# MohamedAtwan/AirCraftOptimalControl

Measured on AMD Instinct MI355X. Metric: Newton iters/sec (whole node), batched 6-state T=500 trajectories; fp64 rel-err, higher is better.
Workload: dtype f64

## Files before the change

### aircraftoptimalcontrol_amd/_lib.py

```python
import ctypes as C
import os
import subprocess

_PKG = os.path.dirname(os.path.abspath(__file__))
_SO = os.environ.get("AOC_LIB") or os.path.join(_PKG, "lib", "libaoc_hip.so")
_SRC = [os.path.join(_PKG, "csrc", f) for f in ("aoc_kernels.hip", "aoc_device.h", "aoc_passes.inc")]
_SRC += sorted(os.path.join(_PKG, "csrc", "passes", f) for f in os.listdir(os.path.join(_PKG, "csrc", "passes")) if f.endswith(".inc"))
_HDR = os.path.join(os.path.dirname(_PKG), "include", "aoc.h")

AOC_TILE = 64
AOC_ENS_NSTAT = 16
AOC_ENV_NREC = 44
AOC_ABI_VERSION = 5

ST_NAN, ST_VNONPOS, ST_SINGULAR, ST_REGULARISED, ST_ARMIJO_EXH, ST_CONVERGED = 1, 2, 4, 8, 16, 32


class AocError(RuntimeError):
    pass


def library_path():
    return _SO


def build_library(force=False, verbose=False):
    deps = _SRC + [_HDR]
    if not force and os.path.exists(_SO) and all(os.path.getmtime(_SO) >= os.path.getmtime(d) for d in deps):
        return _SO
    os.makedirs(os.path.dirname(_SO), exist_ok=True)
    hipcc = os.environ.get("HIPCC", "/opt/rocm/bin/hipcc")
    cmd = [hipcc, "--offload-arch=gfx950", "-O3", "-std=c++17", "-fPIC", "-shared", _SRC[0], "-o", _SO]
    if verbose:
        print(" ".join(cmd))
    subprocess.check_call(cmd)
    return _SO


class Model(C.Structure):
    _fields_ = [(n, C.c_double) for n in ("cd0", "cda", "cla", "m", "g", "S", "rho", "J", "dt")]


class Problem(C.Structure):
    _fields_ = [("model", Model), ("QQt", C.c_double * 36), ("RRt", C.c_double * 4), ("QQT", C.c_double * 36),
                ("B", C.c_int32), ("T", C.c_int32), ("x_in_f32", C.c_int32), ("x_out_f32", C.c_int32),
                ("ref_per_traj", C.c_int32), ("ref_T", C.c_int32), ("x_is_rollout", C.c_int32), ("reserved", C.c_int32),
                ("ref", C.c_void_p), ("stream", C.c_void_p)]


class Params(C.Structure):
    _fields_ = [("max_iters", C.c_int32), ("armijo_maxiters", C.c_int32), ("stepsize_0", C.c_double),
                ("cc", C.c_double), ("beta", C.c_double), ("term_cond", C.c_double),
                ("hessian_switch", C.c_int32), ("reserved", C.c_int32)]


class MpcNoise(C.Structure):
    _fields_ = [("seed", C.c_uint64), ("step", C.c_uint32), ("first", C.c_uint32), ("sigma", C.c_double * 6)]


class Tuning(C.Structure):
    _fields_ = [(n, C.c_int32) for n in ("nspec", "split_tiles", "split_bw_tiles", "fw_lin", "ls_wcap", "ls_kgrow",
                                         "trial_split", "solve_norepack", "ls_worklist", "ls_cpl", "ls_depth_min",
                                         "fw_recompute", "store_candidates", "bw4_tiles", "bw5", "solve_repack_pct",
                                         "solve_sync_fast", "solve_split_tiles", "track_hcut", "bw_hcut", "fw_wpe1",
                                         "hcut_chain6", "bw_hcut_full", "fw_duo", "hcut_waves", "hcut_pairs")]


_P, _I, _D, _Z = C.c_void_p, C.c_int32, C.c_double, C.c_size_t
SYMBOLS = {
    "aoc_get_tuning": (None, [_P]),
    "aoc_set_tuning": (None, [_P]),
    "aoc_version": (C.c_char_p, []),
    "aoc_strerror": (C.c_char_p, [C.c_int]),
    "aoc_last_hip_error": (C.c_char_p, []),
    "aoc_tiled_elems": (_Z, [_I, _I, _I]),
    "aoc_ntiles": (_I, [_I]),
    "aoc_pack": (C.c_int, [_I, _I, _I, _P, _P, _P]),
    "aoc_unpack": (C.c_int, [_I, _I, _I, _P, _P, _P]),
    "aoc_pack_f32": (C.c_int, [_I, _I, _I, _P, _P, _P]),
    "aoc_unpack_f32": (C.c_int, [_I, _I, _I, _P, _P, _P]),
    "aoc_step_batch": (C.c_int, [_P, _I] + [_P] * 10),
    "aoc_cost_batch": (C.c_int, [_P, _I] + [_P] * 10),
    "aoc_traj_cost": (C.c_int, [_P, _P, _P, _P, _P]),
    "aoc_initial_trajectory": (C.c_int, [_P, _D, _D, _P, _P, _P]),
    "aoc_rollout_cost": (C.c_int, [_P] * 9),
    "aoc_backward": (C.c_int, [_P, _I] + [_P] * 7 + [_Z]),
    "aoc_backward_scratch_bytes": (_Z, [_I, _I]),
    "aoc_gradient": (C.c_int, [_P] * 7),
    "aoc_forward": (C.c_int, [_P, _P, _I] + [_P] * 9 + [_Z, _P]),
    "aoc_candidate_bytes": (_Z, [_I, _I, _I]),
    "aoc_default_ncand": (_I, [_I, _I, _I]),
    "aoc_linesearch_scratch_bytes": (_Z, [_I, _I]),
    "aoc_spec_max": (_I, []),
    "aoc_default_nspec": (_I, [_I, _I]),
    "aoc_linesearch": (C.c_int, [_P, _P, _I] + [_P] * 13 + [_Z, _P, _Z]),
    "aoc_linesearch_search": (C.c_int, [_P, _P, _I] + [_P] * 9 + [_Z]),
    "aoc_linesearch_update": (C.c_int, [_P] * 12 + [_Z, _I, _P, _P, _Z]),
    "aoc_lqr_tracking": (C.c_int, [_P] * 9),
    "aoc_ltv_lqr": (C.c_int, [_I, _I, _I] + [_P] * 17),
    "aoc_workspace_bytes": (_Z, [_I, _I]),
    "aoc_newton_iterate": (C.c_int, [_P, _P, _I] + [_P] * 5 + [_Z] + [_P] * 7),
    "aoc_solve_workspace_bytes": (_Z, [_I, _I]),
    "aoc_newton_solve": (C.c_int, [_P] * 6 + [_Z, _I] + [_P] * 10),
    "aoc_newton_solve2": (C.c_int, [_P] * 6 + [_Z, _I] + [_P] * 11),
    "aoc_abi_version": (_I, []),
    "aoc_summary": (C.c_int, [_I, _P, _P, _P, _P, _I, _P]),
    "aoc_streams_concurrent": (C.c_int, [_P, _P]),
    "aoc_solve_trace": (C.c_int, [_P, _I]),
    "aoc_solve_trace_rows": (_I, []),
    "aoc_mpc_step": (C.c_int, [_P] * 3 + [_I] + [_P] * 6 + [_Z] + [_P] * 16),
    "aoc_track_ensemble": (C.c_int, [_P, _I, _I] + [_P] * 8),
    "aoc_ensemble_envelope_scratch_bytes": (_Z, [_I, _I, _I]),
    "aoc_track_ensemble_envelope": (C.c_int, [_P, _I, _I] + [_P] * 10 + [_Z]),
    "aoc_traj_cost_f32": (C.c_int, [_P] * 5),
    "aoc_initial_trajectory_f32": (C.c_int, [_P, _D, _D, _P, _P, _P]),
    "aoc_rollout_cost_f32": (C.c_int, [_P] * 9),
    "aoc_workspace_bytes_f32": (_Z, [_I, _I]),
    "aoc_newton_iterate_f32": (C.c_int, [_P, _P, _I] + [_P] * 5 + [_Z] + [_P] * 7),
# ... 70 lines not shown
```

### aircraftoptimalcontrol_amd/csrc/aoc_kernels.hip

```cpp
#include <hip/hip_runtime.h>

#include <cstdarg>
#include <cstdio>
#include <cstdlib>
#include <cstring>
#include <mutex>
#include <vector>

#include "../../include/aoc.h"

namespace aoc_common {
constexpr int TILE = 64;
}
#define AOC_DEVICE_COMMON
using aoc_common::TILE;

#define AOC_DISPATCH_BOOL(flag, NAME, ...)            \
    do {                                              \
        if (flag) { constexpr bool NAME = true; __VA_ARGS__; } \
        else { constexpr bool NAME = false; __VA_ARGS__; }      \
    } while (0)
#define AOC_DISPATCH_RPT(flag, NAME, ...)                                         \
    do {                                                                          \
        if (flag) { constexpr bool NAME = sizeof(real) == 8; __VA_ARGS__; }       \
// ... 55 lines not shown
    }
    if (lane == 0) { sh[0][wv] = sc; sh[1][wv] = sd; shi[0][wv] = st; shi[1][wv] = nn; }
    __syncthreads();
    if (tid == 0) {
        double a = 0.0, b = 0.0;
        long long c = 0, d = 0;
        for (int w = 0; w < 16; w++) { a += sh[0][w]; b += sh[1][w]; c += shi[0][w]; d += shi[1][w]; }
        if (accumulate) { out[0] += a; out[1] += b; out[2] += (double)c; out[3] += (double)B; out[4] += (double)d; }
        else { out[0] = a; out[1] = b; out[2] = (double)c; out[3] = (double)B; out[4] = (double)d; }
    }
}

__global__ void k_spin(long long ticks, int* sink) {
    const long long t0 = wall_clock64();
    int n = 0;
    while (wall_clock64() - t0 < ticks && n < (1 << 24)) n++;
    if (sink && n < 0) *sink = n;
}

static thread_local char g_hip_err[256] = "";

static int check_launch(const char* what) {
    hipError_t e = hipGetLastError();
    if (e != hipSuccess) {
        snprintf(g_hip_err, sizeof g_hip_err, "%s: %s", what, hipGetErrorString(e));
        return AOC_ELAUNCH;
    }
    return AOC_OK;
}

static int einval(const char* fmt, ...) {
    va_list ap;
    va_start(ap, fmt);
    vsnprintf(g_hip_err, sizeof g_hip_err, fmt, ap);
    va_end(ap);
    return AOC_EINVAL;
}

static aoc_tuning g_tuning;
static std::once_flag g_tuning_once;

static void tuning_defaults(aoc_tuning* t) {
    auto env = [](const char* name, int dflt) { const char* e = getenv(name); return e && *e ? atoi(e) : dflt; };
    memset(t, 0, sizeof *t);
    t->nspec = env("AOC_NSPEC", 0);
    t->split_tiles = env("AOC_SPLIT_TILES", 512);
    t->split_bw_tiles = env("AOC_SPLIT_BW_TILES", 512);
    t->fw_lin = env("AOC_FW_LIN", -1);
    t->ls_wcap = env("AOC_LS_WCAP", 0);
    t->ls_kgrow = env("AOC_LS_KGROW", 0);
    t->trial_split = env("AOC_TRIAL_SPLIT", 1);
    t->solve_norepack = env("AOC_SOLVE_NOREPACK", 0);
    t->ls_worklist = env("AOC_LS_WORKLIST", -1);
    t->ls_cpl = env("AOC_LS_CPL", 1);
    t->ls_depth_min = env("AOC_LS_DEPTH_MIN", 2);
    t->fw_recompute = env("AOC_FW_RECOMPUTE", 1);
    t->store_candidates = env("AOC_STORE_CANDIDATES", 1);
    t->bw4_tiles = env("AOC_BW4_TILES", 256);
    t->bw5 = env("AOC_BW5", 1);
    t->solve_repack_pct = env("AOC_SOLVE_REPACK_PCT", 70);
    t->solve_sync_fast = env("AOC_SOLVE_SYNC_FAST", 2);
    t->solve_split_tiles = env("AOC_SOLVE_SPLIT_TILES", 2048);
    t->track_hcut = env("AOC_TRACK_HCUT", -1);
    t->bw_hcut = env("AOC_BW_HCUT", -1);
    t->fw_wpe1 = env("AOC_FW_WPE1", 1);
    t->hcut_chain6 = env("AOC_HCUT_CHAIN6", 0);
    t->bw_hcut_full = env("AOC_BW_HCUT_FULL", 2);
    t->fw_duo = env("AOC_FW_DUO", 1);
    t->hcut_waves = env("AOC_HCUT_WAVES", 1);
    t->hcut_pairs = env("AOC_HCUT_PAIRS", 1);
}

static const aoc_tuning& tuning() {
    std::call_once(g_tuning_once, [] { tuning_defaults(&g_tuning); });
    return g_tuning;
}

static bool is_diag(const double* M, int n) {
    for (int i = 0; i < n; i++)
        for (int j = 0; j < n; j++)
            if (i != j && M[i * n + j] != 0.0) return false;
    return true;
}

static int check_problem(const aoc_problem* p) {
    if (!p) return einval("aoc_problem is NULL");
    if (!p->ref) return einval("aoc_problem.ref (reference curves) is NULL");
    if (p->B < 1 || p->T < 3) return einval("aoc_problem: B = %d, T = %d (need B >= 1, T >= 3)", p->B, p->T);
    if (p->ref_per_traj && p->ref_T != 0 && p->ref_T < p->T)
        return einval("aoc_problem: ref_T = %d < T = %d (samples per trajectory of the per-trajectory reference array)", p->ref_T, p->T);
    if (p->RRt[1] != p->RRt[2])
        return einval("aoc_problem.RRt is not symmetric (R01 = %g, R10 = %g): the 2x2 gain solve needs R = R^T", p->RRt[1],
                      p->RRt[2]);
    return AOC_OK;
}

static int check_riccati_weights(const aoc_problem* p, const char* who) {
    const struct { const double* M; const char* name; } w[2] = {{p->QQt, "QQt"}, {p->QQT, "QQT"}};
    for (const auto& m : w)
        for (int i = 0; i < 6; i++)
            for (int j = i + 1; j < 6; j++)
                if (m.M[i * 6 + j] != m.M[j * 6 + i])
                    return einval("%s: aoc_problem.%s is not symmetric (%s[%d][%d] = %.17g, %s[%d][%d] = %.17g): the Riccati "
                                  "recursion needs Q = Q^T and Q_T = Q_T^T", who, m.name, m.name, i, j, m.M[i * 6 + j], m.name,
                                  j, i, m.M[j * 6 + i]);
    return AOC_OK;
}
// ... 308 lines not shown
```

### aircraftoptimalcontrol_amd/csrc/passes/api.inc

```
static KConst make_const(const aoc_model& md, const double* Q, const double* R, const double* QT, int B, int T) {
    KConst k;
    memset(&k, 0, sizeof k);
    k.cd0 = (real)md.cd0; k.cda = (real)md.cda; k.cla = (real)md.cla; k.m = (real)md.m; k.g = (real)md.g; k.S = (real)md.S;
    k.rho = (real)md.rho;
    k.J = (real)md.J; k.dt = (real)md.dt;
    k.dtm = (real)(md.dt / md.m);
    k.mg = (real)(md.m * md.g);
    k.hrho = (real)(0.5 * md.rho);
    k.krs = (real)(md.rho * md.S);
    k.b41 = (real)(md.dt / md.J);
    k.rJ = R(1.0) / k.J;
    for (int i = 0; i < 36; i++) { if (Q) k.Q[i] = (real)Q[i]; if (QT) k.QT[i] = (real)QT[i]; }
    for (int i = 0; i < 4; i++) if (R) k.R[i] = (real)R[i];
    k.B = B; k.T = T; k.ntiles = (B + TILE - 1) / TILE;
    k.refT = T; k.rpt = 0;
    k.diag = (Q && R && QT) ? (is_diag(Q, 6) && is_diag(R, 2) && is_diag(QT, 6)) : 1;
    return k;
}

static KConst make_const(const aoc_problem* p) {
    KConst k = make_const(p->model, p->QQt, p->RRt, p->QQT, p->B, p->T);
    k.rpt = p->ref_per_traj != 0;
    if (k.rpt && p->ref_T > 0) k.refT = p->ref_T;
    return k;
// ... 194 lines not shown
    hipLaunchKernelGGL((k_forward<D, RP, N, XR, XT>), dim3(k.ntiles), dim3(TILE), 0, st, k, *prm, (const real*)p->ref, \
                       (const XT*)x, u, x0, Kt, du, descent, J_trial, status)
#define LAUNCH_FW(N)                                                                                                \
    AOC_DISPATCH_DR(k, D, RP, do {                                                                                  \
        if (!p->x_in_f32) LAUNCH_FW_(N, false, real);                                                               \
        else if (xrc) LAUNCH_FW_(N, true, float);                                                                   \
        else LAUNCH_FW_(N, false, float);                                                                           \
    } while (0))
#define LAUNCH_FW_ROLES(KERNEL, GROUPS, NWAVES)                                                                      \
    hipLaunchKernelGGL(KERNEL, dim3(k.ntiles, GROUPS), dim3((NWAVES) * TILE), 0, st, k, *prm, n_spec, cb,           \
                       (const real*)p->ref, (const XT*)x, u, x0, Kt, du, descent, J_trial, status, ntrials_hint)
    const bool xrc = p->x_is_rollout && p->x_in_f32 && tuning().fw_recompute != 0;
    const int split_env = tuning().split_tiles;
    const int split_fw = split_env;
    if (n_spec > 3 || (k.ntiles <= split_fw && p->T >= 3)) {
        if (p->T < 3) return AOC_EINVAL;
        const CandBuf cb = cand_carve(cand, p->B, p->T, n_spec);
        const int one_per_cu = tuning().fw_wpe1 ? 256 : 0;
        const int fw_lin = tuning().fw_lin;
        const int duo_max = tuning().fw_duo == 1 ? 256 : tuning().fw_duo;
        if (duo_max > 0 && n_spec > FWS_TPG && k.ntiles * ((n_spec + 1) / 2) <= duo_max) {
            AOC_DISPATCH_DR(k, D, RP, AOC_DISPATCH_XT(p->x_in_f32, XT,
                LAUNCH_FW_ROLES((k_forward_duo<D, RP, XT>), (n_spec + FWD_CPG - 1) / FWD_CPG, 8)));
        } else if (fw_lin > 0 || (fw_lin < 0 && n_spec <= FWL_TPG)) {
            const int ngroups = (n_spec + FWL_TPG - 1) / FWL_TPG;
            AOC_DISPATCH_DR(k, D, RP, AOC_DISPATCH_XT(p->x_in_f32, XT, AOC_DISPATCH_WPE(k.ntiles * ngroups <= one_per_cu, WPE,
                LAUNCH_FW_ROLES((k_forward_lin<D, RP, XT, WPE>), ngroups, 2 + FWL_TPG))));
        } else {
            const int ngroups = (n_spec + FWS_TPG - 1) / FWS_TPG;
            const int nwaves = 1 + (n_spec < FWS_TPG ? n_spec : FWS_TPG);
            AOC_DISPATCH_DR(k, D, RP, AOC_DISPATCH_XT(p->x_in_f32, XT, AOC_DISPATCH_WPE(k.ntiles * ngroups <= one_per_cu, WPE,
                LAUNCH_FW_ROLES((k_forward_split<D, RP, XT, WPE>), ngroups, nwaves))));
        }
    } else if (n_spec == 1) LAUNCH_FW(1);
    else if (n_spec == 2) LAUNCH_FW(2);
    else LAUNCH_FW(3);
#undef LAUNCH_FW_ROLES
#undef LAUNCH_FW
#undef LAUNCH_FW_
    return check_launch("k_forward");
}

static size_t ls_layout(int ntiles, void* scratch, LsScratch* sc) {
    const size_t nt = (size_t)ntiles;
    size_t off = 0;
    auto take = [&](size_t bytes) { char* q = scratch ? (char*)scratch + off : nullptr; off += align_up(bytes, 16); return q; };
    LsScratch s;
    s.mask = (unsigned long long*)take(nt * sizeof(unsigned long long));
    s.prefix = (int*)take((nt + 1) * sizeof(int));
    s.first_ok = (int*)take(nt * TILE * sizeof(int));
    s.st = (LsState*)take(sizeof(aoc64::LsState));
    s.items = (int2*)take(nt * TILE * LS_WL_IPL * sizeof(int2));
    s.next_r = (int*)take(nt * TILE * sizeof(int));
    s.wl_count = (int*)take(2 * LS_WL_ROUNDS * sizeof(int));
    if (sc) *sc = s;
    return off;
}

static bool ls_use_worklist(int ntiles) {
    const aoc_tuning& tn = tuning();
    return tn.ls_worklist > 0 || (tn.ls_worklist < 0 && ntiles > tn.split_tiles);
}

static int api_ls_search(const aoc_problem* p, const aoc_params* prm, int32_t n_spec, const real* u, const real* x0,
                         const real* du, const real* J_cur, const real* descent, const real* J_trial0, real* stepsize,
                         int32_t* ntrials, void* scratch, size_t scratch_size, LsFrozen frozen = LsFrozen{nullptr, nullptr}) {
    int rc = check_problem(p);
    if (rc) return rc;
    if (!prm || !u || !x0 || !du || !J_cur || !descent || (!J_trial0 && n_spec > 0) || !stepsize || !ntrials || !scratch)
        return einval("aoc_linesearch: NULL argument");
    if (scratch_size < aoc_linesearch_scratch_bytes(p->B, p->T))
        return einval("aoc_linesearch: scratch of %zu bytes, %zu needed (aoc_linesearch_scratch_bytes)", scratch_size,
                      aoc_linesearch_scratch_bytes(p->B, p->T));
    if (prm->armijo_maxiters < 1 || prm->armijo_maxiters >= LS_MAX_STEPS)
        return einval("aoc_linesearch: armijo_maxiters = %d (1 .. %d)", prm->armijo_maxiters, LS_MAX_STEPS - 1);
    if (n_spec < 0 || n_spec > AOC_SPEC_MAX) return einval("aoc_linesearch: n_spec = %d (0 .. %d)", n_spec, AOC_SPEC_MAX);
    KConst k = make_const(p);
    hipStream_t st = (hipStream_t)p->stream;
    LsScratch sc;
    ls_layout(k.ntiles, scratch, &sc);
    const aoc_tuning& tn = tuning();
    if (ls_use_worklist(k.ntiles)) {
        const int cpl = tn.ls_cpl >= 4 ? 4 : tn.ls_cpl >= 2 ? 2 : 1;
        if (prm->armijo_maxiters > 255) return einval("aoc_linesearch: armijo_maxiters > 255");
        const int remaining = prm->armijo_maxiters > n_spec ? prm->armijo_maxiters - n_spec : 0;
        const int per_round = LS_WL_IPL * cpl;
        const int nrounds = remaining > 0 ? 1 + (remaining + per_round - 1) / per_round : 0;
        if (nrounds > LS_WL_ROUNDS)
            return einval("aoc_linesearch: armijo_maxiters = %d needs more than %d work-list rounds", prm->armijo_maxiters,
                          LS_WL_ROUNDS);
        if (hipMemsetAsync(sc.wl_count, 0, 2 * LS_WL_ROUNDS * sizeof(int), st) != hipSuccess)
            return check_launch("aoc_linesearch");
        hipLaunchKernelGGL(k_ls_init_wl, dim3(k.ntiles), dim3(TILE), 0, st, *prm, n_spec, cpl,
                           tn.ls_depth_min > 1 ? tn.ls_depth_min : 1, k.ntiles * TILE, J_cur, descent, J_trial0, stepsize,
                           ntrials, sc, frozen);
        const int ipl = (remaining + cpl - 1) / cpl < LS_WL_IPL ? (remaining + cpl - 1) / cpl : LS_WL_IPL;
        const int wcap = tn.ls_wcap > 0 ? tn.ls_wcap : 2048;
        for (int r = 0; r < nrounds; r++) {
            if (r == 0)
                hipLaunchKernelGGL(k_ls_plan_wl, dim3(k.ntiles), dim3(TILE), 0, st, prm->armijo_maxiters, n_spec, cpl,
                                   wcap * TILE, sc);
            else
                hipLaunchKernelGGL(k_ls_replan, dim3(k.ntiles), dim3(TILE), 0, st, prm->armijo_maxiters, cpl, r, stepsize,
                                   ntrials, sc);
#define LAUNCH_WL(C, PINNED)                                                                                      \
    AOC_DISPATCH_DR(k, D, RP,                                                                                  \
        hipLaunchKernelGGL((k_ls_trial_wl<D, RP, C, PINNED>), dim3(k.ntiles * ipl), dim3(TILE), 0, st, k, *prm, r,    \
                           (const real*)p->ref, u, x0, du, J_cur, descent, sc))
            if (cpl == 4) LAUNCH_WL(4, false);
            else if (cpl == 2) LAUNCH_WL(2, false);
            else {
                LAUNCH_WL(1, true);
                LAUNCH_WL(1, false);
            }
#undef LAUNCH_WL
        }
        return check_launch("aoc_linesearch");
    }
    const int wcap_env = tn.ls_wcap > 0 ? tn.ls_wcap : 1024;
    const int kgrow_set = tn.ls_kgrow;
    const int kgrow_env = kgrow_set > 0 ? kgrow_set : (k.ntiles <= 512 ? 9 : 1);
    const int wcap = k.ntiles > wcap_env ? k.ntiles : wcap_env;
    const bool trial_split = tn.trial_split != 0 && p->T >= 3;
    hipLaunchKernelGGL(k_ls_init, dim3(k.ntiles), dim3(TILE), 0, st, *prm, n_spec, k.ntiles * TILE, J_cur, descent,
                       J_trial0, stepsize, ntrials, sc, frozen);
    const int remaining = prm->armijo_maxiters - n_spec;
    int nrounds = remaining < LS_ROUNDS ? remaining : LS_ROUNDS;
    if (nrounds > 1 && (long)k.ntiles * remaining <= wcap_env && kgrow_env + 1 >= remaining) nrounds = 1;
    for (int r = 0; r < nrounds; r++) {
        const int last = (r == nrounds - 1);
        if (r > 0) hipLaunchKernelGGL(k_ls_resolve, dim3(k.ntiles), dim3(TILE), 0, st, sc, stepsize, ntrials);
        hipLaunchKernelGGL(k_ls_plan, dim3(1), dim3(1024), 0, st, k.ntiles, prm->armijo_maxiters, wcap_env, kgrow_env,
                           last, sc);
        const int grid = last ? k.ntiles * (remaining > 1 ? remaining : 1) : wcap;
        if (trial_split && k.ntiles <= 512) {
            AOC_DISPATCH_DR(k, D, RP,
                hipLaunchKernelGGL((k_ls_trial_split<D, RP>), dim3(grid), dim3(2 * TILE), 0, st, k, *prm, (const real*)p->ref, u,
                                   x0, du, J_cur, descent, sc));
        } else {
            AOC_DISPATCH_DR(k, D, RP,
                hipLaunchKernelGGL((k_ls_trial<D, RP>), dim3(grid), dim3(TILE), 0, st, k, *prm, (const real*)p->ref, u, x0, du,
                                   J_cur, descent, sc));
        }
    }
    return check_launch("aoc_linesearch");
}

static int api_ls_update(const aoc_problem* p, const aoc_params* prm, const real* u, const real* x0, const real* du,
                         void* x_new, real* u_new, real* J_new, real* stepsize, int32_t* ntrials, int32_t* status,
                         void* scratch, size_t scratch_size, int32_t n_spec = 0, const real* J_trial = nullptr,
                         const void* cand = nullptr, size_t cand_size = 0) {
    int rc = check_problem(p);
    if (rc) return rc;
    if (!prm || !u || !x0 || !du || !x_new || !u_new || !J_new || !stepsize || !ntrials || !scratch)
        return einval("aoc_linesearch: NULL argument");
    if (scratch_size < aoc_linesearch_scratch_bytes(p->B, p->T))
        return einval("aoc_linesearch: scratch of %zu bytes, %zu needed (aoc_linesearch_scratch_bytes)", scratch_size,
                      aoc_linesearch_scratch_bytes(p->B, p->T));
    if (cand && J_trial && (n_spec < 1 || n_spec > AOC_SPEC_MAX || cand_size < cand_bytes(p->B, p->T, n_spec)))
        return einval("aoc_linesearch: candidate store of %zu bytes for n_spec = %d, %zu needed (aoc_candidate_bytes)", cand_size,
                      n_spec, n_spec >= 1 && n_spec <= AOC_SPEC_MAX ? cand_bytes(p->B, p->T, n_spec) : (size_t)0);
    if (prm->armijo_maxiters < 1 || prm->armijo_maxiters >= LS_MAX_STEPS)
        return einval("aoc_linesearch: armijo_maxiters = %d (1 .. %d)", prm->armijo_maxiters, LS_MAX_STEPS - 1);
    KConst k = make_const(p);
    hipStream_t st = (hipStream_t)p->stream;
    LsScratch sc;
    ls_layout(k.ntiles, scratch, &sc);
// ... 159 lines not shown
```

### aircraftoptimalcontrol_amd/csrc/passes/linesearch.inc

```
constexpr int LS_MAX_STEPS = 64;
constexpr int LS_NOT_FOUND = 0x7fffffff;
#ifndef AOC_LS_ROUNDS
#define AOC_LS_ROUNDS 4
#endif
constexpr int LS_ROUNDS = AOC_LS_ROUNDS;

constexpr int LS_WL_IPL = 8;
constexpr int LS_WL_ROUNDS = 16;

struct LsState {
    int r_next;
    int r_start;
    int K;
    int count;
    int nw;
    int round;
    int scheme;
    int pad;
    real alpha[LS_MAX_STEPS];
};

struct LsScratch {
    unsigned long long* mask;
    int* prefix;
    int* first_ok;
    LsState* st;
    int2* items;
    int* next_r;
    int* wl_count;
};

struct LsFrozen { const int* orig; const int* ret; };

__global__ __launch_bounds__(TILE) void k_ls_init(aoc_params prm, int nspec, int Bp, const real* __restrict__ J_cur,
                                                  const real* __restrict__ descent,
                                                  const real* __restrict__ J_trial, real* __restrict__ stepsize,
                                                  int* __restrict__ ntrials, LsScratch sc, LsFrozen frozen) {
    const int tile = blockIdx.x, lane = threadIdx.x, b = tile * TILE + lane;
    const real JP = J_cur[b], d = descent[b];
    real a = prm.stepsize_0;
    bool searching = true;
    int ntr = 0;
    real acc = a;
    for (int j = 0; j < nspec && j < prm.armijo_maxiters; j++) {
        if (searching) {
            ntr = j + 1;
            if (!armijo_reject(J_trial[(size_t)j * Bp + b], JP, prm.cc, a, d)) { searching = false; acc = a; }
        }
        a = prm.beta * a;
    }
    if (frozen.orig) {
        const int ob = frozen.orig[b];
        if (ob < 0 || frozen.ret[ob] != -2) { searching = false; acc = R(0.0); ntr = 0; }
    }
    const unsigned long long m = __ballot(searching);
    stepsize[b] = acc;
    ntrials[b] = ntr;
    sc.first_ok[b] = LS_NOT_FOUND;
    if (lane == 0) sc.mask[tile] = m;
    if (tile == 0 && lane == 0) {
        real al = prm.stepsize_0;
        sc.st->alpha[0] = al;
        for (int i = 1; i <= prm.armijo_maxiters; i++) { al = prm.beta * al; sc.st->alpha[i] = al; }
        const int done = nspec < prm.armijo_maxiters ? nspec : prm.armijo_maxiters;
        sc.st->r_next = done;
        sc.st->r_start = done;
        sc.st->K = 0;
        sc.st->count = 0;
        sc.st->nw = 0;
        sc.st->round = 0;
        sc.st->scheme = 0;
// ... 86 lines not shown
    }
}

__device__ __forceinline__ int nth_set_bit(unsigned long long m, int rank) {
    int pos = 0;
#pragma unroll
    for (int w = 32; w >= 1; w >>= 1) {
        const unsigned long long low = m & ((1ull << w) - 1ull);
        const int c = __popcll(low);
        if (rank >= c) { rank -= c; m >>= w; pos += w; }
        else m = low;
    }
    return pos;
}

__device__ __forceinline__ void ls_locate(const LsScratch& sc, int ntiles, int j, int& tile, int& hl) {
    const int* __restrict__ prefix = sc.prefix;
    int lo = 0, hi = ntiles;
    while (hi - lo > 1) {
        const int mid = (lo + hi) >> 1;
        if (prefix[mid] <= j) lo = mid; else hi = mid;
    }
    tile = lo;
    hl = nth_set_bit(sc.mask[lo], j - prefix[lo]);
}

template <bool DIAG, bool RPT>
__global__ __launch_bounds__(TILE) void k_ls_trial(KConst k, aoc_params prm, const real* __restrict__ ref,
                                                   const real* __restrict__ u, const real* __restrict__ x0,
                                                   const real* __restrict__ du, const real* __restrict__ J_cur,
                                                   const real* __restrict__ descent, LsScratch sc) {
    const LsState* st = sc.st;
    const int K = st->K, nw = st->nw;
    const int w = blockIdx.x;
    if (w >= K * nw) return;
    const int kidx = w / nw, slot = w - kidx * nw;
    const int r = st->r_start + kidx;
    const real a_r = st->alpha[r];
    const int count = st->count;
    const int lane = threadIdx.x;
    const int first = slot * TILE;
    const bool valid = first + lane < count;
    int tile, hl;
    ls_locate(sc, k.ntiles, valid ? first + lane : count - 1, tile, hl);
    const int b = tile * TILE + hl;
    real xs[6];
#pragma unroll
    for (int c = 0; c < 6; c++) xs[c] = x0[((size_t)tile * 6 + c) * TILE + hl];
    int f2 = 0;
    const real Jt = rollout<DIAG, RPT, false, real>(k, ref, tile, hl, xs, u, du, a_r, false, nullptr, nullptr, f2);
    if (valid && !armijo_reject(Jt, J_cur[b], prm.cc, a_r, descent[b])) atomicMin(&sc.first_ok[b], r);
}

__device__ __forceinline__ void ls_put_items(const LsScratch& sc, int round, int lane, int b, int r, int depth, int cpl) {
    const int nit = (depth + cpl - 1) / cpl;
    int incl = nit;
#pragma unroll
    for (int off = 1; off < 64; off <<= 1) {
        const int v = __shfl_up(incl, off);
        if (lane >= off) incl += v;
    }
    const int total = __shfl(incl, 63);
    if (total == 0) return;
    int base = 0;
    if (lane == 63) base = atomicAdd(&sc.wl_count[round], total);
    base = __shfl(base, 63);
    int pos = base + incl - nit;
    for (int c = 0; c < nit; c++) {
        const int n = depth - c * cpl < cpl ? depth - c * cpl : cpl;
        sc.items[pos + c] = make_int2(b, (r + c * cpl) | (n << 8));
    }
}

__global__ __launch_bounds__(TILE) void k_ls_init_wl(aoc_params prm, int nspec, int cpl, int depth_min, int Bp,
                                                     const real* __restrict__ J_cur, const real* __restrict__ descent,
                                                     const real* __restrict__ J_trial, real* __restrict__ stepsize,
                                                     int* __restrict__ ntrials, LsScratch sc, LsFrozen frozen) {
    const int tile = blockIdx.x, lane = threadIdx.x, b = tile * TILE + lane;
    const int hint = ntrials[b];
    const real JP = J_cur[b], d = descent[b];
    real a = prm.stepsize_0;
    bool searching = true;
    int ntr = 0;
    real acc = a;
    for (int j = 0; j < nspec && j < prm.armijo_maxiters; j++) {
        if (searching) {
            ntr = j + 1;
            if (!armijo_reject(J_trial[(size_t)j * Bp + b], JP, prm.cc, a, d)) { searching = false; acc = a; }
        }
        a = prm.beta * a;
    }
    if (frozen.orig) {
        const int ob = frozen.orig[b];
        if (ob < 0 || frozen.ret[ob] != -2) { searching = false; acc = R(0.0); ntr = 0; }
    }
    const unsigned long long m = __ballot(searching);
    stepsize[b] = acc;
    ntrials[b] = ntr;
    sc.first_ok[b] = LS_NOT_FOUND;
    if (lane == 0) sc.mask[tile] = m;
    if (tile == 0 && lane == 0) {
        real al = prm.stepsize_0;
        sc.st->alpha[0] = al;
        for (int i = 1; i <= prm.armijo_maxiters; i++) { al = prm.beta * al; sc.st->alpha[i] = al; }
        sc.st->scheme = 1;
    }
    if (m == 0ull) return;
    if (lane == 0) atomicAdd(&sc.wl_count[LS_WL_ROUNDS], __popcll(m));
    const int done = nspec < prm.armijo_maxiters ? nspec : prm.armijo_maxiters;
    const int remaining = prm.armijo_maxiters - done;
    int depth = 0;
    if (searching && remaining > 0) {
        depth = hint >= prm.armijo_maxiters ? remaining : hint - done + 1;
        if (depth < depth_min) depth = depth_min;
        depth = (depth + cpl - 1) / cpl * cpl;
        if (depth > remaining) depth = remaining;
    }
    sc.next_r[b] = depth;
}

__global__ __launch_bounds__(TILE) void k_ls_plan_wl(int maxiters, int nspec, int cpl, int cap_items, LsScratch sc) {
    const int tile = blockIdx.x, lane = threadIdx.x, b = tile * TILE + lane;
    const unsigned long long m = sc.mask[tile];
    if (m == 0ull) return;
    const int done = nspec < maxiters ? nspec : maxiters;
    const int remaining = maxiters - done;
    const bool all = (long)sc.wl_count[LS_WL_ROUNDS] * ((remaining + cpl - 1) / cpl) <= (long)cap_items;
    int depth = 0;
    if ((m >> lane) & 1ull) {
        depth = all ? remaining : sc.next_r[b];
        if (depth > LS_WL_IPL * cpl) depth = LS_WL_IPL * cpl;
        sc.next_r[b] = done + depth;
    }
    ls_put_items(sc, 0, lane, b, done, depth, cpl);
}

__global__ __launch_bounds__(TILE) void k_ls_replan(int maxiters, int cpl, int round, real* __restrict__ stepsize,
                                                    int* __restrict__ ntrials, LsScratch sc) {
    const int tile = blockIdx.x, lane = threadIdx.x, b = tile * TILE + lane;
    const unsigned long long m = sc.mask[tile];
    if (m == 0ull) return;
    bool still = false;
    int depth = 0, r = 0;
    if ((m >> lane) & 1ull) {
        const int f = sc.first_ok[b];
        if (f != LS_NOT_FOUND) { stepsize[b] = sc.st->alpha[f]; ntrials[b] = f + 1; }
        else {
            still = true;
            r = sc.next_r[b];
            depth = maxiters - r;
            if (depth > LS_WL_IPL * cpl) depth = LS_WL_IPL * cpl;
            sc.next_r[b] = r + depth;
        }
    }
    const unsigned long long m2 = __ballot(still);
    if (lane == 0) sc.mask[tile] = m2;
    ls_put_items(sc, round, lane, b, r, depth, cpl);
}

template <bool DIAG, bool RPT, int CPL, int PF = ROLL_PF>
__device__ __forceinline__ void rollout_multi(const KConst& k, const real* __restrict__ ref, int tile, int lane,
                                              const real* __restrict__ x0, const real* __restrict__ u,
                                              const real* __restrict__ du, const real a[CPL], real Jout[CPL],
                                              const TrigK<real>& tk = TrigK<real>()) {
    constexpr int ROLL_PF = PF;
    const int T = k.T;
    real xs[CPL][6], JJ[CPL], q[6], r[2], rb[8];
#pragma unroll
    for (int c = 0; c < 6; c++) {
        const real v = x0[((size_t)tile * 6 + c) * TILE + lane];
#pragma unroll
        for (int j = 0; j < CPL; j++) xs[j][c] = v;
    }
#pragma unroll
    for (int j = 0; j < CPL; j++) JJ[j] = R(0.0);
    real ub[ROLL_PF][2], db[ROLL_PF][2];
#pragma unroll
    for (int i = 0; i < ROLL_PF; i++) {
        const int t = i < T - 1 ? i : T - 2;
        ub[i][0] = u[tix<2>(tile, T, t, 0, lane)];
        ub[i][1] = u[tix<2>(tile, T, t, 1, lane)];
        db[i][0] = du[tix<2>(tile, T, t, 0, lane)];
        db[i][1] = du[tix<2>(tile, T, t, 1, lane)];
    }
    for (int t0 = 0; t0 < T - 1; t0 += ROLL_PF) {
#pragma unroll
        for (int i = 0; i < ROLL_PF; i++) {
            const int t = t0 + i;
            if (t >= T - 1) break;
            const real uc0 = ring_take(ub[i][0]), uc1 = ring_take(ub[i][1]), dc0 = ring_take(db[i][0]), dc1 = ring_take(db[i][1]);
            {
                const int tn = t + ROLL_PF < T - 1 ? t + ROLL_PF : T - 2;
                ub[i][0] = u[tix<2>(tile, T, tn, 0, lane)];
                ub[i][1] = u[tix<2>(tile, T, tn, 1, lane)];
                db[i][0] = du[tix<2>(tile, T, tn, 0, lane)];
                db[i][1] = du[tix<2>(tile, T, tn, 1, lane)];
            }
            const real* rr = ref_row<RPT>(k, ref, tile, lane, t, rb);
#pragma unroll
            for (int j = 0; j < CPL; j++) {
                real u0, u1, xn[6];
                step_inputs(uc0, uc1, a[j], dc0, dc1, u0, u1);
                JJ[j] += stage_cost2<DIAG>(k, xs[j], u0, u1, rr, q, r);
                const SC s = trig(xs[j][3], xs[j][5], tk);
                step_state(k, xs[j], u0, u1, s, xn);
#pragma unroll
                for (int c = 0; c < 6; c++) xs[j][c] = xn[c];
            }
        }
    }
#pragma unroll
    for (int j = 0; j < CPL; j++) {
        JJ[j] += term_cost2<DIAG>(k, xs[j], ref_row<RPT>(k, ref, tile, lane, T - 1, rb), q);
        Jout[j] = R(0.5) * JJ[j];
    }
}

template <bool DIAG, bool RPT, int CPL, int PF = ROLL_PF>
__device__ __forceinline__ void ls_trial_item(const KConst& k, const aoc_params& prm, const real* __restrict__ ref,
                                              const real* __restrict__ u, const real* __restrict__ x0,
                                              const real* __restrict__ du, const real* __restrict__ J_cur,
                                              const real* __restrict__ descent, const LsScratch& sc, int b, int r0, int n,
                                              const TrigK<real>& tk = TrigK<real>()) {
    real a[CPL], J[CPL];
#pragma unroll
    for (int j = 0; j < CPL; j++) a[j] = sc.st->alpha[r0 + (j < n ? j : 0)];
    rollout_multi<DIAG, RPT, CPL, PF>(k, ref, b / TILE, b % TILE, x0, u, du, a, J, tk);
    if (n <= 0) return;
    const real JP = J_cur[b], d = descent[b];
    int acc = -1;
#pragma unroll
    for (int j = CPL - 1; j >= 0; j--)
        if (j < n && !armijo_reject(J[j], JP, prm.cc, a[j], d)) acc = j;
    if (acc >= 0) atomicMin(&sc.first_ok[b], r0 + acc);
}

#ifndef AOC_LS_WL_PIN_ITEMS
#define AOC_LS_WL_PIN_ITEMS (1024 * TILE)
#endif
constexpr int LS_WL_PIN_ITEMS = AOC_LS_WL_PIN_ITEMS;
#ifndef AOC_LS_WL_PF
#define AOC_LS_WL_PF 8
#endif
constexpr int LS_WL_PF = AOC_LS_WL_PF;
template <bool DIAG, bool RPT, int CPL, bool PIN>
__global__ __launch_bounds__(TILE) void k_ls_trial_wl(KConst kc, aoc_params prm, int round, const real* __restrict__ ref,
                                                      const real* __restrict__ u, const real* __restrict__ x0,
                                                      const real* __restrict__ du, const real* __restrict__ J_cur,
                                                      const real* __restrict__ descent, LsScratch sc) {
    const int count = sc.wl_count[round];
    const int first = blockIdx.x * TILE, lane = threadIdx.x;
    if (first >= count || (CPL == 1 && PIN != (count <= LS_WL_PIN_ITEMS))) return;
    KConst k = kc;
    TrigK<real> tk;
    if (PIN) { pin_consts<DIAG>(k); pin_trig(tk); }
    const bool valid = first + lane < count;
    const int2 it = sc.items[valid ? first + lane : count - 1];
    ls_trial_item<DIAG, RPT, CPL, (PIN ? ROLL_PF : LS_WL_PF)>(k, prm, ref, u, x0, du, J_cur, descent, sc, it.x, it.y & 0xff,
                                                               valid ? it.y >> 8 : 0, tk);
}

template <bool DIAG, bool RPT, typename XO>
__global__ __launch_bounds__(TILE) void k_ls_final(KConst k, int maxiters, const real* __restrict__ ref,
                                                   const real* __restrict__ u, const real* __restrict__ x0,
                                                   const real* __restrict__ du, XO* __restrict__ x_new,
                                                   real* __restrict__ u_new, real* __restrict__ J_new,
                                                   real* __restrict__ stepsize, int* __restrict__ ntrials,
                                                   int* __restrict__ status, LsScratch sc) {
    const int tile = blockIdx.x, lane = threadIdx.x, b = tile * TILE + lane;
    const LsState* st = sc.st;
    int flags = 0;
    const unsigned long long m = sc.mask[tile];
    if (m != 0ull) {
        const unsigned long long left = st->scheme ? ls_resolve_wl(m, b, st, sc.first_ok, stepsize, ntrials, lane)
                                         : (st->K > 0) ? ls_resolve(m, b, st->r_next, st, sc.first_ok, stepsize, ntrials, lane) : m;
        if ((left >> lane) & 1ull) {
            stepsize[b] = st->alpha[maxiters];
            ntrials[b] = maxiters;
            flags |= AOC_ST_ARMIJO_EXH;
        }
    }
    const real a = stepsize[b];
    real xs[6];
#pragma unroll
    for (int c = 0; c < 6; c++) xs[c] = x0[((size_t)tile * 6 + c) * TILE + lane];
    const real Jf = rollout<DIAG, RPT, true, XO>(k, ref, tile, lane, xs, u, du, a, true, x_new, u_new, flags);
    if (Jf != Jf || Jf - Jf != R(0.0)) flags |= AOC_ST_NAN;
    J_new[b] = Jf;
    if (status && flags) status[b] |= flags;
}

template <bool DIAG, bool RPT, typename XO, bool WRITE = true, int SHIFT = 0>
__device__ __forceinline__ real rollout_split(const KConst& k, const real* __restrict__ ref, int tile, int lane, bool chain,
                                              real a, const real* __restrict__ x0, const real* __restrict__ u,
                                              const real* __restrict__ du, XO* __restrict__ x_new,
                                              real* __restrict__ u_new, real (*sh)[4][TILE][2], int& flags, int ll = -1,
                                              const TrigK<real>& tk = TrigK<real>(), const real* xs0 = nullptr) {
    const int T = k.T;
    if (ll < 0) ll = lane;
    if (chain) {
        real xs[6], xn[6];
#pragma unroll
        for (int c = 0; c < 6; c++) {
            xs[c] = xs0 ? xs0[c] : x0[((size_t)tile * 6 + c) * TILE + lane];
            if (WRITE) x_new[tix<6>(tile, T, 0, c, lane)] = (XO)xs[c];
        }
        const bool has_du = du != nullptr;
        const real* __restrict__ dsrc = has_du ? du : u;
        real ub[ROLL_PF][2], db[ROLL_PF][2];
#pragma unroll
        for (int i = 0; i < ROLL_PF; i++) {
            const int t = i + SHIFT < T - 1 ? i + SHIFT : T - 2;
// ... 203 lines not shown
```

Measured before the change: 20.37 million.

## Choose line-search chains-per-lane per round from predicted work-list crowding

Line-search work-list rounds now pick chains-per-lane and the pinned versus unpinned trial kernel on the device, per round. The choice uses a predicted candidate count that init and trial kernels accumulate with wave reductions and atomics, replacing a fixed host-side cpl. The multi-chain rollout also splits trigonometry into a fast path plus a rare fix-up for huge angles. This aims to match kernel variant to occupancy and cut wasted rollouts, at the cost of extra atomics, more launches per round, and a default tuning change to the adaptive rule.

```diff
diff --git a/aircraftoptimalcontrol_amd/_lib.py b/aircraftoptimalcontrol_amd/_lib.py
--- a/aircraftoptimalcontrol_amd/_lib.py
+++ b/aircraftoptimalcontrol_amd/_lib.py
@@ -64,6 +64,12 @@
                                          "fw_recompute", "store_candidates", "bw4_tiles", "bw5", "solve_repack_pct",
                                          "solve_sync_fast", "solve_split_tiles", "track_hcut", "bw_hcut", "fw_wpe1",
                                          "hcut_chain6", "bw_hcut_full", "fw_duo", "hcut_waves", "hcut_pairs")]
+
+
+def ls_cpl_rule(chains=None, crowded_items=None):
+    c = {None: 0, 1: 1, 2: 2, 4: 3}[chains]
+    n = 0 if crowded_items is None else int(crowded_items) + 1
+    return -1 - (c + 4 * n)
 
 
 _P, _I, _D, _Z = C.c_void_p, C.c_int32, C.c_double, C.c_size_t
diff --git a/aircraftoptimalcontrol_amd/csrc/aoc_kernels.hip b/aircraftoptimalcontrol_amd/csrc/aoc_kernels.hip
--- a/aircraftoptimalcontrol_amd/csrc/aoc_kernels.hip
+++ b/aircraftoptimalcontrol_amd/csrc/aoc_kernels.hip
@@ -131,7 +131,7 @@
     t->trial_split = env("AOC_TRIAL_SPLIT", 1);
     t->solve_norepack = env("AOC_SOLVE_NOREPACK", 0);
     t->ls_worklist = env("AOC_LS_WORKLIST", -1);
-    t->ls_cpl = env("AOC_LS_CPL", 1);
+    t->ls_cpl = env("AOC_LS_CPL", -1);
     t->ls_depth_min = env("AOC_LS_DEPTH_MIN", 2);
     t->fw_recompute = env("AOC_FW_RECOMPUTE", 1);
     t->store_candidates = env("AOC_STORE_CANDIDATES", 1);
diff --git a/aircraftoptimalcontrol_amd/csrc/passes/api.inc b/aircraftoptimalcontrol_amd/csrc/passes/api.inc
--- a/aircraftoptimalcontrol_amd/csrc/passes/api.inc
+++ b/aircraftoptimalcontrol_amd/csrc/passes/api.inc
@@ -270,7 +270,7 @@
     s.st = (LsState*)take(sizeof(aoc64::LsState));
     s.items = (int2*)take(nt * TILE * LS_WL_IPL * sizeof(int2));
     s.next_r = (int*)take(nt * TILE * sizeof(int));
-    s.wl_count = (int*)take(2 * LS_WL_ROUNDS * sizeof(int));
+    s.wl_count = (int*)take(3 * LS_WL_ROUNDS * sizeof(int));
     if (sc) *sc = s;
     return off;
 }
@@ -278,6 +278,14 @@
 static bool ls_use_worklist(int ntiles) {
     const aoc_tuning& tn = tuning();
     return tn.ls_worklist > 0 || (tn.ls_worklist < 0 && ntiles > tn.split_tiles);
+}
+
+static LsRegime ls_regime(int ls_cpl) {
+    if (ls_cpl >= 4) return LsRegime{4, 4, -1};
+    if (ls_cpl >= 2) return LsRegime{2, 2, -1};
+    if (ls_cpl >= 0) return LsRegime{1, 1, LS_WL_PIN_ITEMS};
+    const int v = -1 - ls_cpl, code = v & 3, thr = v >> 2;
+    return LsRegime{1, code == 3 ? 4 : code ? code : LS_WL_CPL_CROWDED, thr ? thr - 1 : LS_WL_PIN_ITEMS};
 }
 
 static int api_ls_search(const aoc_problem* p, const aoc_params* prm, int32_t n_spec, const real* u, const real* x0,
@@ -299,38 +307,36 @@
     ls_layout(k.ntiles, scratch, &sc);
     const aoc_tuning& tn = tuning();
     if (ls_use_worklist(k.ntiles)) {
-        const int cpl = tn.ls_cpl >= 4 ? 4 : tn.ls_cpl >= 2 ? 2 : 1;
+        const LsRegime rg = ls_regime(tn.ls_cpl);
         if (prm->armijo_maxiters > 255) return einval("aoc_linesearch: armijo_maxiters > 255");
         const int remaining = prm->armijo_maxiters > n_spec ? prm->armijo_maxiters - n_spec : 0;
-        const int per_round = LS_WL_IPL * cpl;
+        const int per_round = LS_WL_IPL * rg.cpl_lone;
         const int nrounds = remaining > 0 ? 1 + (remaining + per_round - 1) / per_round : 0;
         if (nrounds > LS_WL_ROUNDS)
             return einval("aoc_linesearch: armijo_maxiters = %d needs more than %d work-list rounds", prm->armijo_maxiters,
                           LS_WL_ROUNDS);
-        if (hipMemsetAsync(sc.wl_count, 0, 2 * LS_WL_ROUNDS * sizeof(int), st) != hipSuccess)
+        if (hipMemsetAsync(sc.wl_count, 0, 3 * LS_WL_ROUNDS * sizeof(int), st) != hipSuccess)
             return check_launch("aoc_linesearch");
-        hipLaunchKernelGGL(k_ls_init_wl, dim3(k.ntiles), dim3(TILE), 0, st, *prm, n_spec, cpl,
+        hipLaunchKernelGGL(k_ls_init_wl, dim3(k.ntiles), dim3(TILE), 0, st, *prm, n_spec,
                            tn.ls_depth_min > 1 ? tn.ls_depth_min : 1, k.ntiles * TILE, J_cur, descent, J_trial0, stepsize,
                            ntrials, sc, frozen);
-        const int ipl = (remaining + cpl - 1) / cpl < LS_WL_IPL ? (remaining + cpl - 1) / cpl : LS_WL_IPL;
         const int wcap = tn.ls_wcap > 0 ? tn.ls_wcap : 2048;
         for (int r = 0; r < nrounds; r++) {
             if (r == 0)
-                hipLaunchKernelGGL(k_ls_plan_wl, dim3(k.ntiles), dim3(TILE), 0, st, prm->armijo_maxiters, n_spec, cpl,
+                hipLaunchKernelGGL(k_ls_plan_wl, dim3(k.ntiles), dim3(TILE), 0, st, prm->armijo_maxiters, n_spec, rg,
                                    wcap * TILE, sc);
             else
-                hipLaunchKernelGGL(k_ls_replan, dim3(k.ntiles), dim3(TILE), 0, st, prm->armijo_maxiters, cpl, r, stepsize,
+                hipLaunchKernelGGL(k_ls_replan, dim3(k.ntiles), dim3(TILE), 0, st, prm->armijo_maxiters, rg, r, stepsize,
                                    ntrials, sc);
 #define LAUNCH_WL(C, PINNED)                                                                                      \
     AOC_DISPATCH_DR(k, D, RP,                                                                                  \
-        hipLaunchKernelGGL((k_ls_trial_wl<D, RP, C, PINNED>), dim3(k.ntiles * ipl), dim3(TILE), 0, st, k, *prm, r,    \
-                           (const real*)p->ref, u, x0, du, J_cur, descent, sc))
-            if (cpl == 4) LAUNCH_WL(4, false);
-            else if (cpl == 2) LAUNCH_WL(2, false);
-            else {
-                LAUNCH_WL(1, true);
-                LAUNCH_WL(1, false);
-            }
+        hipLaunchKernelGGL((k_ls_trial_wl<D, RP, C, PINNED>),                                                          \
+                           dim3(k.ntiles * (((remaining + C - 1) / C < LS_WL_IPL) ? (remaining + C - 1) / C : LS_WL_IPL)),  \
+                           dim3(TILE), 0, st, k, *prm, r, (const real*)p->ref, u, x0, du, J_cur, descent, sc))
+            if (rg.cpl_lone == 1) LAUNCH_WL(1, true);
+            if (rg.cpl_crowded == 4) LAUNCH_WL(4, false);
+            else if (rg.cpl_crowded == 2) LAUNCH_WL(2, false);
+            else LAUNCH_WL(1, false);
 #undef LAUNCH_WL
         }
         return check_launch("aoc_linesearch");
diff --git a/aircraftoptimalcontrol_amd/csrc/passes/linesearch.inc b/aircraftoptimalcontrol_amd/csrc/passes/linesearch.inc
--- a/aircraftoptimalcontrol_amd/csrc/passes/linesearch.inc
+++ b/aircraftoptimalcontrol_amd/csrc/passes/linesearch.inc
@@ -16,7 +16,8 @@
     int nw;
     int round;
     int scheme;
-    int pad;
+    int crowded;
+    int cpl[LS_WL_ROUNDS];
     real alpha[LS_MAX_STEPS];
 };
 
@@ -209,6 +210,24 @@
     if (valid && !armijo_reject(Jt, J_cur[b], prm.cc, a_r, descent[b])) atomicMin(&sc.first_ok[b], r);
 }
 
+struct LsRegime { int cpl_lone, cpl_crowded, crowded_items; };
+
+__device__ __forceinline__ int ls_choose_regime(const LsScratch& sc, const LsRegime& rg, int round, long cands, bool record) {
+    const bool crowded = cands > (long)rg.crowded_items;
+    const int cpl = crowded ? rg.cpl_crowded : rg.cpl_lone;
+    if (record) {
+        sc.st->cpl[round] = cpl;
+        sc.st->crowded = ((round ? sc.st->crowded : 0) & ~(1 << round)) | ((int)crowded << round);
+    }
+    return cpl;
+}
+
+__device__ __forceinline__ int ls_wave_sum(int v) {
+#pragma unroll
+    for (int o = TILE / 2; o > 0; o >>= 1) v += __shfl_xor(v, o);
+    return v;
+}
+
 __device__ __forceinline__ void ls_put_items(const LsScratch& sc, int round, int lane, int b, int r, int depth, int cpl) {
     const int nit = (depth + cpl - 1) / cpl;
     int incl = nit;
@@ -229,7 +248,7 @@
     }
 }
 
-__global__ __launch_bounds__(TILE) void k_ls_init_wl(aoc_params prm, int nspec, int cpl, int depth_min, int Bp,
+__global__ __launch_bounds__(TILE) void k_ls_init_wl(aoc_params prm, int nspec, int depth_min, int Bp,
                                                      const real* __restrict__ J_cur, const real* __restrict__ descent,
                                                      const real* __restrict__ J_trial, real* __restrict__ stepsize,
                                                      int* __restrict__ ntrials, LsScratch sc, LsFrozen frozen) {
@@ -270,31 +289,37 @@
     if (searching && remaining > 0) {
         depth = hint >= prm.armijo_maxiters ? remaining : hint - done + 1;
         if (depth < depth_min) depth = depth_min;
-        depth = (depth + cpl - 1) / cpl * cpl;
         if (depth > remaining) depth = remaining;
     }
     sc.next_r[b] = depth;
-}
-
-__global__ __launch_bounds__(TILE) void k_ls_plan_wl(int maxiters, int nspec, int cpl, int cap_items, LsScratch sc) {
+    const int pred = ls_wave_sum(depth < LS_WL_IPL ? depth : LS_WL_IPL);
+    if (lane == 0) atomicAdd(&sc.wl_count[2 * LS_WL_ROUNDS], pred);
+}
+
+__global__ __launch_bounds__(TILE) void k_ls_plan_wl(int maxiters, int nspec, LsRegime rg, int cap_items, LsScratch sc) {
     const int tile = blockIdx.x, lane = threadIdx.x, b = tile * TILE + lane;
+    const int done = nspec < maxiters ? nspec : maxiters;
+    const int remaining = maxiters - done;
+    const long searching = sc.wl_count[LS_WL_ROUNDS];
+    const bool all = searching * ((remaining + rg.cpl_lone - 1) / rg.cpl_lone) <= (long)cap_items;
+    const long cands = all ? searching * (remaining < LS_WL_IPL ? remaining : LS_WL_IPL) : (long)sc.wl_count[2 * LS_WL_ROUNDS];
+    const int cpl = ls_choose_regime(sc, rg, 0, cands, tile == 0 && lane == 0);
     const unsigned long long m = sc.mask[tile];
     if (m == 0ull) return;
-    const int done = nspec < maxiters ? nspec : maxiters;
-    const int remaining = maxiters - done;
-    const bool all = (long)sc.wl_count[LS_WL_ROUNDS] * ((remaining + cpl - 1) / cpl) <= (long)cap_items;
     int depth = 0;
     if ((m >> lane) & 1ull) {
-        depth = all ? remaining : sc.next_r[b];
+        depth = all ? remaining : (sc.next_r[b] + cpl - 1) / cpl * cpl;
+        if (depth > remaining) depth = remaining;
         if (depth > LS_WL_IPL * cpl) depth = LS_WL_IPL * cpl;
         sc.next_r[b] = done + depth;
     }
     ls_put_items(sc, 0, lane, b, done, depth, cpl);
 }
 
-__global__ __launch_bounds__(TILE) void k_ls_replan(int maxiters, int cpl, int round, real* __restrict__ stepsize,
+__global__ __launch_bounds__(TILE) void k_ls_replan(int maxiters, LsRegime rg, int round, real* __restrict__ stepsize,
                                                     int* __restrict__ ntrials, LsScratch sc) {
     const int tile = blockIdx.x, lane = threadIdx.x, b = tile * TILE + lane;
+    const int cpl = ls_choose_regime(sc, rg, round, sc.wl_count[2 * LS_WL_ROUNDS + round], tile == 0 && lane == 0);
     const unsigned long long m = sc.mask[tile];
     if (m == 0ull) return;
     bool still = false;
@@ -354,13 +379,24 @@
                 db[i][1] = du[tix<2>(tile, T, tn, 1, lane)];
             }
             const real* rr = ref_row<RPT>(k, ref, tile, lane, t, rb);
+            real u0[CPL], u1[CPL];
+            SC s[CPL];
+            bool huge = false;
 #pragma unroll
             for (int j = 0; j < CPL; j++) {
-                real u0, u1, xn[6];
-                step_inputs(uc0, uc1, a[j], dc0, dc1, u0, u1);
-                JJ[j] += stage_cost2<DIAG>(k, xs[j], u0, u1, rr, q, r);
-                const SC s = trig(xs[j][3], xs[j][5], tk);
-                step_state(k, xs[j], u0, u1, s, xn);
+                step_inputs(uc0, uc1, a[j], dc0, dc1, u0[j], u1[j]);
+                JJ[j] += stage_cost2<DIAG>(k, xs[j], u0[j], u1[j], rr, q, r);
+                s[j] = trig_fast(xs[j][3], xs[j][5], tk);
+                huge = huge || trig_huge(xs[j][3], xs[j][5]);
+            }
+            if (huge) {
+#pragma unroll
+                for (int j = 0; j < CPL; j++) trig_fix(xs[j][3], xs[j][5], s[j]);
+            }
+#pragma unroll
+            for (int j = 0; j < CPL; j++) {
+                real xn[6];
+                step_state(k, xs[j], u0[j], u1[j], s[j], xn);
 #pragma unroll
                 for (int c = 0; c < 6; c++) xs[j][c] = xn[c];
             }
@@ -377,19 +413,27 @@
 __device__ __forceinline__ void ls_trial_item(const KConst& k, const aoc_params& prm, const real* __restrict__ ref,
                                               const real* __restrict__ u, const real* __restrict__ x0,
                                               const real* __restrict__ du, const real* __restrict__ J_cur,
-                                              const real* __restrict__ descent, const LsScratch& sc, int b, int r0, int n,
-                                              const TrigK<real>& tk = TrigK<real>()) {
+                                              const real* __restrict__ descent, const LsScratch& sc, int round, int b, int r0,
+                                              int n, const TrigK<real>& tk = TrigK<real>()) {
     real a[CPL], J[CPL];
 #pragma unroll
     for (int j = 0; j < CPL; j++) a[j] = sc.st->alpha[r0 + (j < n ? j : 0)];
+    int rest = 0;
+    if (n > 0 && r0 + n == sc.next_r[b]) {
+        rest = prm.armijo_maxiters - (r0 + n);
+        if (rest > LS_WL_IPL) rest = LS_WL_IPL;
+    }
     rollout_multi<DIAG, RPT, CPL, PF>(k, ref, b / TILE, b % TILE, x0, u, du, a, J, tk);
-    if (n <= 0) return;
-    const real JP = J_cur[b], d = descent[b];
-    int acc = -1;
-#pragma unroll
-    for (int j = CPL - 1; j >= 0; j--)
-        if (j < n && !armijo_reject(J[j], JP, prm.cc, a[j], d)) acc = j;
-    if (acc >= 0) atomicMin(&sc.first_ok[b], r0 + acc);
+    if (n > 0) {
+        const real JP = J_cur[b], d = descent[b];
+        int acc = -1;
+#pragma unroll
+        for (int j = CPL - 1; j >= 0; j--)
+            if (j < n && !armijo_reject(J[j], JP, prm.cc, a[j], d)) acc = j;
+        if (acc >= 0) { atomicMin(&sc.first_ok[b], r0 + acc); rest = 0; }
+    }
+    rest = ls_wave_sum(rest);
+    if (threadIdx.x == 0 && rest > 0 && round + 1 < LS_WL_ROUNDS) atomicAdd(&sc.wl_count[2 * LS_WL_ROUNDS + round + 1], rest);
 }
 
 #ifndef AOC_LS_WL_PIN_ITEMS
@@ -400,6 +444,10 @@
 #define AOC_LS_WL_PF 8
 #endif
 constexpr int LS_WL_PF = AOC_LS_WL_PF;
+#ifndef AOC_LS_WL_CPL_CROWDED
+#define AOC_LS_WL_CPL_CROWDED 1
+#endif
+constexpr int LS_WL_CPL_CROWDED = AOC_LS_WL_CPL_CROWDED;
 template <bool DIAG, bool RPT, int CPL, bool PIN>
 __global__ __launch_bounds__(TILE) void k_ls_trial_wl(KConst kc, aoc_params prm, int round, const real* __restrict__ ref,
                                                       const real* __restrict__ u, const real* __restrict__ x0,
@@ -407,14 +455,14 @@
                                                       const real* __restrict__ descent, LsScratch sc) {
     const int count = sc.wl_count[round];
     const int first = blockIdx.x * TILE, lane = threadIdx.x;
-    if (first >= count || (CPL == 1 && PIN != (count <= LS_WL_PIN_ITEMS))) return;
+    if (first >= count || sc.st->cpl[round] != CPL || PIN == (bool)((sc.st->crowded >> round) & 1)) return;
     KConst k = kc;
     TrigK<real> tk;
     if (PIN) { pin_consts<DIAG>(k); pin_trig(tk); }
     const bool valid = first + lane < count;
     const int2 it = sc.items[valid ? first + lane : count - 1];
-    ls_trial_item<DIAG, RPT, CPL, (PIN ? ROLL_PF : LS_WL_PF)>(k, prm, ref, u, x0, du, J_cur, descent, sc, it.x, it.y & 0xff,
-                                                               valid ? it.y >> 8 : 0, tk);
+    ls_trial_item<DIAG, RPT, CPL, (PIN ? ROLL_PF : LS_WL_PF)>(k, prm, ref, u, x0, du, J_cur, descent, sc, round, it.x,
+                                                               it.y & 0xff, valid ? it.y >> 8 : 0, tk);
 }
 
 template <bool DIAG, bool RPT, typename XO>
```

New measurement: 20.37 million, median of 2. No clear change (+0.0%).
